# 3DOM-FBK/deep-image-matching

Measured on NVIDIA H100. Metric: image-pairs/sec (SuperPoint+LightGlue, 1024x1024, 2048 kpts), higher is better.
Workload: dtype f16 hi/lo split x3 MMA, f32 accumulate (fp32-class)

## Files before the change

deep-image-matching_b200/csrc/attention.cuh:

```cuda
#pragma once
#include "common.cuh"
#include "sm90.cuh"

namespace {

constexpr int kAttnBlk = 64;
constexpr int kAttnTile = 128;
constexpr int kAttnThreads = 9 * 32;

template <int HD, bool SPLIT>
struct AttnGeom {
  static constexpr int kPl = SPLIT ? 2 : 1;
  static constexpr int kAtoms = HD / 64;
  static constexpr int kAtomQ = kAttnTile * 128, kQB = kAtoms * kAtomQ;
  static constexpr int kAtomK = kAttnBlk * 128, kKB = kAtoms * kAtomK;
  static constexpr int kVB = HD * 128;
  static constexpr int kSmem = kPl * (kQB + 2 * (kKB + kVB)) + 256 + 1024;
};

template <int HD, bool SPLIT, class Out>
__device__ __forceinline__ void attn_tile(const CUtensorMap* tmQh, const CUtensorMap* tmQl, const CUtensorMap* tmKh,
                                          const CUtensorMap* tmKl, const CUtensorMap* tmVh, const CUtensorMap* tmVl, int qrow, int krow,
                                          int vrow, int nq, int nk, float scale, float lazy, const Out& out) {
  using namespace sm90;
  using G = AttnGeom<HD, SPLIT>;
  extern __shared__ uint8_t sm_attn_raw[];
  uint8_t* smem = sm_attn_raw + ((1024u - (smem_u32(sm_attn_raw) & 1023u)) & 1023u);
  uint8_t* sQ = smem;
  uint8_t* sK = sQ + G::kPl * G::kQB;
  uint8_t* sV = sK + 2 * G::kPl * G::kKB;
  uint64_t* bars = reinterpret_cast<uint64_t*>(sV + 2 * G::kPl * G::kVB);
  uint64_t *bQ = bars, *kFull = bars + 1, *kEmpty = bars + 3, *vFull = bars + 5, *vEmpty = bars + 7;
  const int tid = threadIdx.x, warp = tid >> 5, lane = tid & 31;
  if (tid == 0) {
    mbar_init(bQ, 1);
    for (int i = 0; i < 2; ++i) {
      mbar_init(&kFull[i], 1);
      mbar_init(&kEmpty[i], 8);
      mbar_init(&vFull[i], 1);
      mbar_init(&vEmpty[i], 8);
    }
    fence_barrier_init();
  }
  __syncthreads();
  const int nblk = (nk + kAttnBlk - 1) / kAttnBlk;

  if (warp == 8) {
    if (nblk > 0 && elect_one()) {
      mbar_expect_tx(bQ, G::kPl * G::kQB);
      for (int at = 0; at < G::kAtoms; ++at) {
        tma_load_2d(sQ + at * G::kAtomQ, tmQh, bQ, at * 64, qrow);
        if (SPLIT) tma_load_2d(sQ + G::kQB + at * G::kAtomQ, tmQl, bQ, at * 64, qrow);
      }
    }
    __syncwarp();
    for (int j = 0; j < nblk; ++j) {
      const int s = j & 1;
      const uint32_t ph = (j >> 1) & 1;
      mbar_wait(&kEmpty[s], ph ^ 1);
      if (elect_one()) {
        mbar_expect_tx(&kFull[s], G::kPl * G::kKB);
        for (int at = 0; at < G::kAtoms; ++at) {
          tma_load_2d(sK + s * G::kPl * G::kKB + at * G::kAtomK, tmKh, &kFull[s], at * 64, krow + j * kAttnBlk);
          if (SPLIT) tma_load_2d(sK + s * G::kPl * G::kKB + G::kKB + at * G::kAtomK, tmKl, &kFull[s], at * 64, krow + j * kAttnBlk);
        }
      }
      __syncwarp();
      mbar_wait(&vEmpty[s], ph ^ 1);
      if (elect_one()) {
        mbar_expect_tx(&vFull[s], G::kPl * G::kVB);
        tma_load_2d(sV + s * G::kPl * G::kVB, tmVh, &vFull[s], j * kAttnBlk, vrow);
        if (SPLIT) tma_load_2d(sV + s * G::kPl * G::kVB + G::kVB, tmVl, &vFull[s], j * kAttnBlk, vrow);
      }
      __syncwarp();
    }
    return;
  }
  const int wg = warp >> 2, w4 = warp & 3;
  const int r0 = 64 * wg + 16 * w4 + (lane >> 2);
  const uint32_t q_wg = smem_u32(sQ) + wg * 64 * 128;
  float o[HD / 2];
#pragma unroll
  for (int i = 0; i < HD / 2; ++i) o[i] = 0.f;
  float m_run[2] = {-INFINITY, -INFINITY}, l_run[2] = {0.f, 0.f};
  const float c2 = scale * 1.4426950408889634f;
  if (nblk > 0) mbar_wait(bQ, 0);
  for (int j = 0; j < nblk; ++j) {
    const int s = j & 1;
    const uint32_t ph = (j >> 1) & 1;
    float sc[kAttnBlk / 2];
    mbar_wait(&kFull[s], ph);
    {
      const uint32_t kb = smem_u32(sK + s * G::kPl * G::kKB);
      wgmma_fence();
#pragma unroll
      for (int kk = 0; kk < 4 * G::kAtoms; ++kk) {
        const uint64_t qh = sdesc_advance_k(make_sdesc_sw128(q_wg + (kk >> 2) * G::kAtomQ), kk & 3);
        const uint64_t kh = sdesc_advance_k(make_sdesc_sw128(kb + (kk >> 2) * G::kAtomK), kk & 3);
        Wgmma<kAttnBlk>::ss(sc, qh, kh, kk != 0);
        if (SPLIT) {
          const uint64_t ql = sdesc_advance_k(make_sdesc_sw128(q_wg + G::kQB + (kk >> 2) * G::kAtomQ), kk & 3);
          const uint64_t kl = sdesc_advance_k(make_sdesc_sw128(kb + G::kKB + (kk >> 2) * G::kAtomK), kk & 3);
          Wgmma<kAttnBlk>::ss(sc, qh, kl, 1);
          Wgmma<kAttnBlk>::ss(sc, ql, kh, 1);
        }
      }
      wgmma_commit();
      wgmma_wait<0>();
      wgmma_fence_regs(sc);
    }
    if (lane == 0) mbar_arrive(&kEmpty[s]);
    const int key0 = j * kAttnBlk + 2 * (lane & 3);
    if (j * kAttnBlk + kAttnBlk > nk) {
#pragma unroll
      for (int i = 0; i < kAttnBlk / 8; ++i)
#pragma unroll
        for (int e = 0; e < 4; ++e)
          if (key0 + 8 * i + (e & 1) >= nk) sc[4 * i + e] = -INFINITY;
    }
    float alpha[2], mc[2];
#pragma unroll
    for (int h = 0; h < 2; ++h) {
      float mx = sc[2 * h];
#pragma unroll
      for (int i = 0; i < kAttnBlk / 8; ++i) mx = fmaxf(mx, fmaxf(sc[4 * i + 2 * h], sc[4 * i + 2 * h + 1]));
      mx = fmaxf(mx, __shfl_xor_sync(0xffffffffu, mx, 1));
      mx = fmaxf(mx, __shfl_xor_sync(0xffffffffu, mx, 2));
      const float m_blk = fmaxf(m_run[h], mx);
      const bool grow = (m_blk - m_run[h]) * c2 > lazy;
      const float m_new = grow ? m_blk : m_run[h];
      alpha[h] = grow ? fast_exp2((m_run[h] - m_new) * c2) : 1.f;
      mc[h] = m_new * c2;
      m_run[h] = m_new;
    }
    float ps[2] = {0.f, 0.f};
#pragma unroll
    for (int i = 0; i < kAttnBlk / 8; ++i)
#pragma unroll
      for (int e = 0; e < 4; ++e) {
        sc[4 * i + e] = fast_exp2(fmaf(sc[4 * i + e], c2, -mc[e >> 1]));
        ps[e >> 1] += sc[4 * i + e];
      }
#pragma unroll
    for (int h = 0; h < 2; ++h) l_run[h] = l_run[h] * alpha[h] + ps[h];
#pragma unroll
    for (int i = 0; i < HD / 8; ++i) {
      o[4 * i] *= alpha[0], o[4 * i + 1] *= alpha[0];
      o[4 * i + 2] *= alpha[1], o[4 * i + 3] *= alpha[1];
    }
    uint32_t ph_[kAttnBlk / 4], pl_[kAttnBlk / 4];
#pragma unroll
    for (int c = 0; c < kAttnBlk / 4; ++c) {
      __half2 h2, l2;
      split2_f32(sc[2 * c], sc[2 * c + 1], h2, l2);
      ph_[c] = *reinterpret_cast<uint32_t*>(&h2);
      pl_[c] = *reinterpret_cast<uint32_t*>(&l2);
    }
    mbar_wait(&vFull[s], ph);
    {
      const uint32_t vb = smem_u32(sV + s * G::kPl * G::kVB);
      const uint64_t v_h = make_sdesc_sw128(vb), v_l = make_sdesc_sw128(vb + G::kVB);
      wgmma_fence();
#pragma unroll
      for (int kk = 0; kk < kAttnBlk / 16; ++kk) {
        const uint32_t ah[4] = {ph_[4 * kk], ph_[4 * kk + 1], ph_[4 * kk + 2], ph_[4 * kk + 3]};
        Wgmma<HD>::rs(o, ah, sdesc_advance_k(v_h, kk), 1);
        if (SPLIT) {
          const uint32_t al[4] = {pl_[4 * kk], pl_[4 * kk + 1], pl_[4 * kk + 2], pl_[4 * kk + 3]};
          Wgmma<HD>::rs(o, ah, sdesc_advance_k(v_l, kk), 1);
          Wgmma<HD>::rs(o, al, sdesc_advance_k(v_h, kk), 1);
        }
      }
      wgmma_commit();
      wgmma_wait<0>();
      wgmma_fence_regs(o);
    }
    if (lane == 0) mbar_arrive(&vEmpty[s]);
  }
  float inv[2];
#pragma unroll
  for (int h = 0; h < 2; ++h) {
    float l = l_run[h];
    l += __shfl_xor_sync(0xffffffffu, l, 1);
    l += __shfl_xor_sync(0xffffffffu, l, 2);
    inv[h] = nblk > 0 ? 1.f / l : 0.f;
  }
#pragma unroll
  for (int i = 0; i < HD / 8; ++i) {
    const int col = 8 * i + 2 * (lane & 3);
    if (r0 < nq) out(r0, col, o[4 * i] * inv[0], o[4 * i + 1] * inv[0]);
    if (r0 + 8 < nq) out(r0 + 8, col, o[4 * i + 2] * inv[1], o[4 * i + 3] * inv[1]);
  }
}

}
```

deep-image-matching_b200/csrc/sm90.cuh:

```cuda
#pragma once
#include <cuda.h>
#include <cuda_fp16.h>
#include <cuda_runtime.h>
#include <stdint.h>

namespace sm90 {

__device__ __forceinline__ uint32_t smem_u32(const void* p) {
  return static_cast<uint32_t>(__cvta_generic_to_shared(p));
}

__device__ __forceinline__ void mbar_init(uint64_t* bar, uint32_t count) {
  asm volatile("mbarrier.init.shared::cta.b64 [%0], %1;" ::"r"(smem_u32(bar)), "r"(count) : "memory");
}
__device__ __forceinline__ void fence_barrier_init() {
  asm volatile("fence.mbarrier_init.release.cluster;" ::: "memory");
}
__device__ __forceinline__ void mbar_expect_tx(uint64_t* bar, uint32_t bytes) {
  asm volatile("mbarrier.arrive.expect_tx.shared::cta.b64 _, [%0], %1;" ::"r"(smem_u32(bar)), "r"(bytes) : "memory");
}
__device__ __forceinline__ void mbar_arrive(uint64_t* bar) {
  asm volatile("mbarrier.arrive.shared::cta.b64 _, [%0];" ::"r"(smem_u32(bar)) : "memory");
}
__device__ __forceinline__ bool mbar_try_wait(uint64_t* bar, uint32_t parity) {
  uint32_t ok;
  asm volatile(
      "{\n\t.reg .pred p;\n\t"
      "mbarrier.try_wait.parity.shared::cta.b64 p, [%1], %2;\n\t"
      "selp.u32 %0, 1, 0, p;\n\t}"
      : "=r"(ok)
      : "r"(smem_u32(bar)), "r"(parity)
      : "memory");
  return ok != 0;
}
__device__ __forceinline__ void mbar_wait(uint64_t* bar, uint32_t parity) {
  if (mbar_try_wait(bar, parity)) return;
  uint32_t polls = 0;
  long long t0 = 0;
  while (!mbar_try_wait(bar, parity)) {
    if ((++polls & 0x3ffu) == 0) {
      const long long now = clock64();
      if (t0 == 0) t0 = now;
      if (now - t0 > 8000000000LL) {
        __trap();
      }
    }
  }
}

__device__ __forceinline__ float fast_exp2(float x) {
  float y;
  asm("ex2.approx.ftz.f32 %0, %1;" : "=f"(y) : "f"(x));
  return y;
}

__device__ __forceinline__ bool elect_one() {
  uint32_t pred;
  asm volatile(
      "{\n\t.reg .pred p;\n\t"
      "elect.sync _|p, 0xffffffff;\n\t"
      "selp.u32 %0, 1, 0, p;\n\t}"
      : "=r"(pred));
  return pred != 0;
}

__device__ __forceinline__ void fence_proxy_async_smem() {
  asm volatile("fence.proxy.async.shared::cta;" ::: "memory");
}
template <int N>
__device__ __forceinline__ void setmaxnreg_dec() {
  asm volatile("setmaxnreg.dec.sync.aligned.u32 %0;" ::"n"(N));
}
template <int N>
__device__ __forceinline__ void setmaxnreg_inc() {
  asm volatile("setmaxnreg.inc.sync.aligned.u32 %0;" ::"n"(N));
}
__device__ __forceinline__ void named_bar_sync(int id, int threads) {
  asm volatile("bar.sync %0, %1;" ::"r"(id), "r"(threads) : "memory");
}

__device__ __forceinline__ void tma_prefetch_desc(const CUtensorMap* m) {
  asm volatile("prefetch.tensormap [%0];" ::"l"(reinterpret_cast<uint64_t>(m)) : "memory");
}
__device__ __forceinline__ void tma_load_2d(void* dst, const CUtensorMap* m, uint64_t* bar, int c0, int c1) {
  asm volatile(
      "cp.async.bulk.tensor.2d.shared::cluster.global.mbarrier::complete_tx::bytes [%0], [%1, {%3, %4}], [%2];" ::"r"(
          smem_u32(dst)),
      "l"(reinterpret_cast<uint64_t>(m)), "r"(smem_u32(bar)), "r"(c0), "r"(c1)
      : "memory");
}
__device__ __forceinline__ void tma_load_4d(void* dst, const CUtensorMap* m, uint64_t* bar, int c0, int c1, int c2, int c3) {
  asm volatile(
      "cp.async.bulk.tensor.4d.shared::cluster.global.mbarrier::complete_tx::bytes [%0], [%1, {%3, %4, %5, %6}], [%2];" ::
          "r"(smem_u32(dst)),
      "l"(reinterpret_cast<uint64_t>(m)), "r"(smem_u32(bar)), "r"(c0), "r"(c1), "r"(c2), "r"(c3)
      : "memory");
}

__device__ __forceinline__ void tma_prefetch_2d(const CUtensorMap* m, int c0, int c1) {
  asm volatile("cp.async.bulk.prefetch.tensor.2d.L2.global.tile [%0, {%1, %2}];" ::"l"(reinterpret_cast<uint64_t>(m)), "r"(c0), "r"(c1)
               : "memory");
}
__device__ __forceinline__ void tma_prefetch_4d(const CUtensorMap* m, int c0, int c1, int c2, int c3) {
  asm volatile("cp.async.bulk.prefetch.tensor.4d.L2.global.tile [%0, {%1, %2, %3, %4}];" ::"l"(reinterpret_cast<uint64_t>(m)), "r"(c0),
               "r"(c1), "r"(c2), "r"(c3)
               : "memory");
}

constexpr uint32_t kLayoutSw128 = 1, kLayoutSw64 = 2;
__device__ __forceinline__ uint64_t make_sdesc(uint32_t saddr, uint32_t sbo_bytes, uint32_t layout) {
  uint64_t d = 0;
  d |= static_cast<uint64_t>((saddr & 0x3FFFFu) >> 4);
  d |= static_cast<uint64_t>(1) << 16;
  d |= static_cast<uint64_t>(sbo_bytes >> 4) << 32;
  d |= static_cast<uint64_t>(layout) << 62;
  return d;
}
__device__ __forceinline__ uint64_t make_sdesc_sw128(uint32_t saddr) { return make_sdesc(saddr, 1024, kLayoutSw128); }
__device__ __forceinline__ uint64_t sdesc_advance_k(uint64_t d, int k16) { return d + static_cast<uint64_t>(k16 * 2); }

__device__ __forceinline__ void wgmma_fence() { asm volatile("wgmma.fence.sync.aligned;" ::: "memory"); }
__device__ __forceinline__ void wgmma_commit() { asm volatile("wgmma.commit_group.sync.aligned;" ::: "memory"); }
template <int N>
__device__ __forceinline__ void wgmma_wait() {
  asm volatile("wgmma.wait_group.sync.aligned %0;" ::"n"(N) : "memory");
}
template <int N>
__device__ __forceinline__ void wgmma_fence_regs(float (&d)[N]) {
#pragma unroll
  for (int i = 0; i < N; ++i) asm volatile("" : "+f"(d[i])::"memory");
}

template <int N>
struct Wgmma;

template <>
struct Wgmma<64> {
  static __device__ __forceinline__ void ss(float* d, uint64_t a, uint64_t b, int scale_d) {
    asm volatile(
        "{\n\t.reg .pred p;\n\t"
        "setp.ne.b32 p, %34, 0;\n\t"
        "wgmma.mma_async.sync.aligned.m64n64k16.f32.f16.f16 {%0, %1, %2, %3, %4, %5, %6, %7, %8, %9, %10, %11, %12, %13, %14, %15, %16, %17, %18, %19, %20, %21, %22, %23, %24, %25, %26, %27, %28, %29, %30, %31}, %32, %33, p, 1, 1, 0, 0;\n\t}"
        : "+f"(d[0]), "+f"(d[1]), "+f"(d[2]), "+f"(d[3]), "+f"(d[4]), "+f"(d[5]), "+f"(d[6]), "+f"(d[7]), "+f"(d[8]), "+f"(d[9]), "+f"(d[10]), "+f"(d[11]), "+f"(d[12]), "+f"(d[13]), "+f"(d[14]), "+f"(d[15]), "+f"(d[16]), "+f"(d[17]), "+f"(d[18]), "+f"(d[19]), "+f"(d[20]), "+f"(d[21]), "+f"(d[22]), "+f"(d[23]), "+f"(d[24]), "+f"(d[25]), "+f"(d[26]), "+f"(d[27]), "+f"(d[28]), "+f"(d[29]), "+f"(d[30]), "+f"(d[31])
        : "l"(a), "l"(b), "r"(scale_d));
  }
  static __device__ __forceinline__ void rs(float* d, const uint32_t (&a)[4], uint64_t b, int scale_d) {
    asm volatile(
        "{\n\t.reg .pred p;\n\t"
        "setp.ne.b32 p, %37, 0;\n\t"
        "wgmma.mma_async.sync.aligned.m64n64k16.f32.f16.f16 {%0, %1, %2, %3, %4, %5, %6, %7, %8, %9, %10, %11, %12, %13, %14, %15, %16, %17, %18, %19, %20, %21, %22, %23, %24, %25, %26, %27, %28, %29, %30, %31}, {%32, %33, %34, %35}, %36, p, 1, 1, 0;\n\t}"
        : "+f"(d[0]), "+f"(d[1]), "+f"(d[2]), "+f"(d[3]), "+f"(d[4]), "+f"(d[5]), "+f"(d[6]), "+f"(d[7]), "+f"(d[8]), "+f"(d[9]), "+f"(d[10]), "+f"(d[11]), "+f"(d[12]), "+f"(d[13]), "+f"(d[14]), "+f"(d[15]), "+f"(d[16]), "+f"(d[17]), "+f"(d[18]), "+f"(d[19]), "+f"(d[20]), "+f"(d[21]), "+f"(d[22]), "+f"(d[23]), "+f"(d[24]), "+f"(d[25]), "+f"(d[26]), "+f"(d[27]), "+f"(d[28]), "+f"(d[29]), "+f"(d[30]), "+f"(d[31])
        : "r"(a[0]), "r"(a[1]), "r"(a[2]), "r"(a[3]), "l"(b), "r"(scale_d));
  }
};

template <>
struct Wgmma<128> {
  static __device__ __forceinline__ void ss(float* d, uint64_t a, uint64_t b, int scale_d) {
    asm volatile(
        "{\n\t.reg .pred p;\n\t"
        "setp.ne.b32 p, %66, 0;\n\t"
        "wgmma.mma_async.sync.aligned.m64n128k16.f32.f16.f16 {%0, %1, %2, %3, %4, %5, %6, %7, %8, %9, %10, %11, %12, %13, %14, %15, %16, %17, %18, %19, %20, %21, %22, %23, %24, %25, %26, %27, %28, %29, %30, %31, %32, %33, %34, %35, %36, %37, %38, %39, %40, %41, %42, %43, %44, %45, %46, %47, %48, %49, %50, %51, %52, %53, %54, %55, %56, %57, %58, %59, %60, %61, %62, %63}, %64, %65, p, 1, 1, 0, 0;\n\t}"
        : "+f"(d[0]), "+f"(d[1]), "+f"(d[2]), "+f"(d[3]), "+f"(d[4]), "+f"(d[5]), "+f"(d[6]), "+f"(d[7]), "+f"(d[8]), "+f"(d[9]), "+f"(d[10]), "+f"(d[11]), "+f"(d[12]), "+f"(d[13]), "+f"(d[14]), "+f"(d[15]), "+f"(d[16]), "+f"(d[17]), "+f"(d[18]), "+f"(d[19]), "+f"(d[20]), "+f"(d[21]), "+f"(d[22]), "+f"(d[23]), "+f"(d[24]), "+f"(d[25]), "+f"(d[26]), "+f"(d[27]), "+f"(d[28]), "+f"(d[29]), "+f"(d[30]), "+f"(d[31]), "+f"(d[32]), "+f"(d[33]), "+f"(d[34]), "+f"(d[35]), "+f"(d[36]), "+f"(d[37]), "+f"(d[38]), "+f"(d[39]), "+f"(d[40]), "+f"(d[41]), "+f"(d[42]), "+f"(d[43]), "+f"(d[44]), "+f"(d[45]), "+f"(d[46]), "+f"(d[47]), "+f"(d[48]), "+f"(d[49]), "+f"(d[50]), "+f"(d[51]), "+f"(d[52]), "+f"(d[53]), "+f"(d[54]), "+f"(d[55]), "+f"(d[56]), "+f"(d[57]), "+f"(d[58]), "+f"(d[59]), "+f"(d[60]), "+f"(d[61]), "+f"(d[62]), "+f"(d[63])
        : "l"(a), "l"(b), "r"(scale_d));
  }
  static __device__ __forceinline__ void rs(float* d, const uint32_t (&a)[4], uint64_t b, int scale_d) {
    asm volatile(
        "{\n\t.reg .pred p;\n\t"
        "setp.ne.b32 p, %69, 0;\n\t"
        "wgmma.mma_async.sync.aligned.m64n128k16.f32.f16.f16 {%0, %1, %2, %3, %4, %5, %6, %7, %8, %9, %10, %11, %12, %13, %14, %15, %16, %17, %18, %19, %20, %21, %22, %23, %24, %25, %26, %27, %28, %29, %30, %31, %32, %33, %34, %35, %36, %37, %38, %39, %40, %41, %42, %43, %44, %45, %46, %47, %48, %49, %50, %51, %52, %53, %54, %55, %56, %57, %58, %59, %60, %61, %62, %63}, {%64, %65, %66, %67}, %68, p, 1, 1, 0;\n\t}"
        : "+f"(d[0]), "+f"(d[1]), "+f"(d[2]), "+f"(d[3]), "+f"(d[4]), "+f"(d[5]), "+f"(d[6]), "+f"(d[7]), "+f"(d[8]), "+f"(d[9]), "+f"(d[10]), "+f"(d[11]), "+f"(d[12]), "+f"(d[13]), "+f"(d[14]), "+f"(d[15]), "+f"(d[16]), "+f"(d[17]), "+f"(d[18]), "+f"(d[19]), "+f"(d[20]), "+f"(d[21]), "+f"(d[22]), "+f"(d[23]), "+f"(d[24]), "+f"(d[25]), "+f"(d[26]), "+f"(d[27]), "+f"(d[28]), "+f"(d[29]), "+f"(d[30]), "+f"(d[31]), "+f"(d[32]), "+f"(d[33]), "+f"(d[34]), "+f"(d[35]), "+f"(d[36]), "+f"(d[37]), "+f"(d[38]), "+f"(d[39]), "+f"(d[40]), "+f"(d[41]), "+f"(d[42]), "+f"(d[43]), "+f"(d[44]), "+f"(d[45]), "+f"(d[46]), "+f"(d[47]), "+f"(d[48]), "+f"(d[49]), "+f"(d[50]), "+f"(d[51]), "+f"(d[52]), "+f"(d[53]), "+f"(d[54]), "+f"(d[55]), "+f"(d[56]), "+f"(d[57]), "+f"(d[58]), "+f"(d[59]), "+f"(d[60]), "+f"(d[61]), "+f"(d[62]), "+f"(d[63])
        : "r"(a[0]), "r"(a[1]), "r"(a[2]), "r"(a[3]), "l"(b), "r"(scale_d));
  }
};

template <>
struct Wgmma<256> {
  static __device__ __forceinline__ void ss(float* d, uint64_t a, uint64_t b, int scale_d) {
    asm volatile(
        "{\n\t.reg .pred p;\n\t"
        "setp.ne.b32 p, %130, 0;\n\t"
        "wgmma.mma_async.sync.aligned.m64n256k16.f32.f16.f16 {%0, %1, %2, %3, %4, %5, %6, %7, %8, %9, %10, %11, %12, %13, %14, %15, %16, %17, %18, %19, %20, %21, %22, %23, %24, %25, %26, %27, %28, %29, %30, %31, %32, %33, %34, %35, %36, %37, %38, %39, %40, %41, %42, %43, %44, %45, %46, %47, %48, %49, %50, %51, %52, %53, %54, %55, %56, %57, %58, %59, %60, %61, %62, %63, %64, %65, %66, %67, %68, %69, %70, %71, %72, %73, %74, %75, %76, %77, %78, %79, %80, %81, %82, %83, %84, %85, %86, %87, %88, %89, %90, %91, %92, %93, %94, %95, %96, %97, %98, %99, %100, %101, %102, %103, %104, %105, %106, %107, %108, %109, %110, %111, %112, %113, %114, %115, %116, %117, %118, %119, %120, %121, %122, %123, %124, %125, %126, %127}, %128, %129, p, 1, 1, 0, 0;\n\t}"
        : "+f"(d[0]), "+f"(d[1]), "+f"(d[2]), "+f"(d[3]), "+f"(d[4]), "+f"(d[5]), "+f"(d[6]), "+f"(d[7]), "+f"(d[8]), "+f"(d[9]), "+f"(d[10]), "+f"(d[11]), "+f"(d[12]), "+f"(d[13]), "+f"(d[14]), "+f"(d[15]), "+f"(d[16]), "+f"(d[17]), "+f"(d[18]), "+f"(d[19]), "+f"(d[20]), "+f"(d[21]), "+f"(d[22]), "+f"(d[23]), "+f"(d[24]), "+f"(d[25]), "+f"(d[26]), "+f"(d[27]), "+f"(d[28]), "+f"(d[29]), "+f"(d[30]), "+f"(d[31]), "+f"(d[32]), "+f"(d[33]), "+f"(d[34]), "+f"(d[35]), "+f"(d[36]), "+f"(d[37]), "+f"(d[38]), "+f"(d[39]), "+f"(d[40]), "+f"(d[41]), "+f"(d[42]), "+f"(d[43]), "+f"(d[44]), "+f"(d[45]), "+f"(d[46]), "+f"(d[47]), "+f"(d[48]), "+f"(d[49]), "+f"(d[50]), "+f"(d[51]), "+f"(d[52]), "+f"(d[53]), "+f"(d[54]), "+f"(d[55]), "+f"(d[56]), "+f"(d[57]), "+f"(d[58]), "+f"(d[59]), "+f"(d[60]), "+f"(d[61]), "+f"(d[62]), "+f"(d[63]), "+f"(d[64]), "+f"(d[65]), "+f"(d[66]), "+f"(d[67]), "+f"(d[68]), "+f"(d[69]), "+f"(d[70]), "+f"(d[71]), "+f"(d[72]), "+f"(d[73]), "+f"(d[74]), "+f"(d[75]), "+f"(d[76]), "+f"(d[77]), "+f"(d[78]), "+f"(d[79]), "+f"(d[80]), "+f"(d[81]), "+f"(d[82]), "+f"(d[83]), "+f"(d[84]), "+f"(d[85]), "+f"(d[86]), "+f"(d[87]), "+f"(d[88]), "+f"(d[89]), "+f"(d[90]), "+f"(d[91]), "+f"(d[92]), "+f"(d[93]), "+f"(d[94]), "+f"(d[95]), "+f"(d[96]), "+f"(d[97]), "+f"(d[98]), "+f"(d[99]), "+f"(d[100]), "+f"(d[101]), "+f"(d[102]), "+f"(d[103]), "+f"(d[104]), "+f"(d[105]), "+f"(d[106]), "+f"(d[107]), "+f"(d[108]), "+f"(d[109]), "+f"(d[110]), "+f"(d[111]), "+f"(d[112]), "+f"(d[113]), "+f"(d[114]), "+f"(d[115]), "+f"(d[116]), "+f"(d[117]), "+f"(d[118]), "+f"(d[119]), "+f"(d[120]), "+f"(d[121]), "+f"(d[122]), "+f"(d[123]), "+f"(d[124]), "+f"(d[125]), "+f"(d[126]), "+f"(d[127])
        : "l"(a), "l"(b), "r"(scale_d));
  }
  static __device__ __forceinline__ void rs(float* d, const uint32_t (&a)[4], uint64_t b, int scale_d) {
    asm volatile(
        "{\n\t.reg .pred p;\n\t"
        "setp.ne.b32 p, %133, 0;\n\t"
        "wgmma.mma_async.sync.aligned.m64n256k16.f32.f16.f16 {%0, %1, %2, %3, %4, %5, %6, %7, %8, %9, %10, %11, %12, %13, %14, %15, %16, %17, %18, %19, %20, %21, %22, %23, %24, %25, %26, %27, %28, %29, %30, %31, %32, %33, %34, %35, %36, %37, %38, %39, %40, %41, %42, %43, %44, %45, %46, %47, %48, %49, %50, %51, %52, %53, %54, %55, %56, %57, %58, %59, %60, %61, %62, %63, %64, %65, %66, %67, %68, %69, %70, %71, %72, %73, %74, %75, %76, %77, %78, %79, %80, %81, %82, %83, %84, %85, %86, %87, %88, %89, %90, %91, %92, %93, %94, %95, %96, %97, %98, %99, %100, %101, %102, %103, %104, %105, %106, %107, %108, %109, %110, %111, %112, %113, %114, %115, %116, %117, %118, %119, %120, %121, %122, %123, %124, %125, %126, %127}, {%128, %129, %130, %131}, %132, p, 1, 1, 0;\n\t}"
        : "+f"(d[0]), "+f"(d[1]), "+f"(d[2]), "+f"(d[3]), "+f"(d[4]), "+f"(d[5]), "+f"(d[6]), "+f"(d[7]), "+f"(d[8]), "+f"(d[9]), "+f"(d[10]), "+f"(d[11]), "+f"(d[12]), "+f"(d[13]), "+f"(d[14]), "+f"(d[15]), "+f"(d[16]), "+f"(d[17]), "+f"(d[18]), "+f"(d[19]), "+f"(d[20]), "+f"(d[21]), "+f"(d[22]), "+f"(d[23]), "+f"(d[24]), "+f"(d[25]), "+f"(d[26]), "+f"(d[27]), "+f"(d[28]), "+f"(d[29]), "+f"(d[30]), "+f"(d[31]), "+f"(d[32]), "+f"(d[33]), "+f"(d[34]), "+f"(d[35]), "+f"(d[36]), "+f"(d[37]), "+f"(d[38]), "+f"(d[39]), "+f"(d[40]), "+f"(d[41]), "+f"(d[42]), "+f"(d[43]), "+f"(d[44]), "+f"(d[45]), "+f"(d[46]), "+f"(d[47]), "+f"(d[48]), "+f"(d[49]), "+f"(d[50]), "+f"(d[51]), "+f"(d[52]), "+f"(d[53]), "+f"(d[54]), "+f"(d[55]), "+f"(d[56]), "+f"(d[57]), "+f"(d[58]), "+f"(d[59]), "+f"(d[60]), "+f"(d[61]), "+f"(d[62]), "+f"(d[63]), "+f"(d[64]), "+f"(d[65]), "+f"(d[66]), "+f"(d[67]), "+f"(d[68]), "+f"(d[69]), "+f"(d[70]), "+f"(d[71]), "+f"(d[72]), "+f"(d[73]), "+f"(d[74]), "+f"(d[75]), "+f"(d[76]), "+f"(d[77]), "+f"(d[78]), "+f"(d[79]), "+f"(d[80]), "+f"(d[81]), "+f"(d[82]), "+f"(d[83]), "+f"(d[84]), "+f"(d[85]), "+f"(d[86]), "+f"(d[87]), "+f"(d[88]), "+f"(d[89]), "+f"(d[90]), "+f"(d[91]), "+f"(d[92]), "+f"(d[93]), "+f"(d[94]), "+f"(d[95]), "+f"(d[96]), "+f"(d[97]), "+f"(d[98]), "+f"(d[99]), "+f"(d[100]), "+f"(d[101]), "+f"(d[102]), "+f"(d[103]), "+f"(d[104]), "+f"(d[105]), "+f"(d[106]), "+f"(d[107]), "+f"(d[108]), "+f"(d[109]), "+f"(d[110]), "+f"(d[111]), "+f"(d[112]), "+f"(d[113]), "+f"(d[114]), "+f"(d[115]), "+f"(d[116]), "+f"(d[117]), "+f"(d[118]), "+f"(d[119]), "+f"(d[120]), "+f"(d[121]), "+f"(d[122]), "+f"(d[123]), "+f"(d[124]), "+f"(d[125]), "+f"(d[126]), "+f"(d[127])
        : "r"(a[0]), "r"(a[1]), "r"(a[2]), "r"(a[3]), "l"(b), "r"(scale_d));
  }
};

__device__ __forceinline__ uint32_t sw128_offset(int row, int col) {
  return static_cast<uint32_t>(row * 128 + ((((col >> 3) ^ row) & 7) << 4) + ((col & 7) << 1));
}

}
```

Baseline: 221.9.

## Pipeline attention S and PV wgmmas with ping-pong warpgroup scheduling

Restructures the attention consumer loop in FlashAttention-3 style. Each iteration now issues the QK^T wgmma for block j together with the PV wgmma for block j-1, so the softmax of block j runs while the PV matmul is still in flight. Named barriers make the two warpgroups alternate their MMA issue, Q is held in registers via ldmatrix when the head dim is 64, and the O rescale is skipped when no row max changed. It also adds an early exit when there are no keys. The cost is higher register pressure from the extra live fragments, plus barrier coordination that could serialize or deadlock if the warpgroups' block counts diverge.

After: 227.7 (median of 6 runs). +2.6%, better.

```diff
diff --git a/deep-image-matching_b200/csrc/attention.cuh b/deep-image-matching_b200/csrc/attention.cuh
--- a/deep-image-matching_b200/csrc/attention.cuh
+++ b/deep-image-matching_b200/csrc/attention.cuh
@@ -16,6 +16,7 @@
   static constexpr int kAtomK = kAttnBlk * 128, kKB = kAtoms * kAtomK;
   static constexpr int kVB = HD * 128;
   static constexpr int kSmem = kPl * (kQB + 2 * (kKB + kVB)) + 256 + 1024;
+  static constexpr bool kQReg = HD == 64;
 };
 
 template <int HD, bool SPLIT, class Out>
@@ -78,38 +79,76 @@
   }
   const int wg = warp >> 2, w4 = warp & 3;
   const int r0 = 64 * wg + 16 * w4 + (lane >> 2);
-  const uint32_t q_wg = smem_u32(sQ) + wg * 64 * 128;
   float o[HD / 2];
 #pragma unroll
   for (int i = 0; i < HD / 2; ++i) o[i] = 0.f;
   float m_run[2] = {-INFINITY, -INFINITY}, l_run[2] = {0.f, 0.f};
   const float c2 = scale * 1.4426950408889634f;
-  if (nblk > 0) mbar_wait(bQ, 0);
-  for (int j = 0; j < nblk; ++j) {
-    const int s = j & 1;
-    const uint32_t ph = (j >> 1) & 1;
-    float sc[kAttnBlk / 2];
-    mbar_wait(&kFull[s], ph);
-    {
-      const uint32_t kb = smem_u32(sK + s * G::kPl * G::kKB);
-      wgmma_fence();
-#pragma unroll
-      for (int kk = 0; kk < 4 * G::kAtoms; ++kk) {
+  if (nblk == 0) {
+#pragma unroll
+    for (int i = 0; i < HD / 8; ++i) {
+      const int col = 8 * i + 2 * (lane & 3);
+      if (r0 < nq) out(r0, col, 0.f, 0.f);
+      if (r0 + 8 < nq) out(r0 + 8, col, 0.f, 0.f);
+    }
+    return;
+  }
+  const uint32_t q_wg = smem_u32(sQ) + wg * 64 * 128;
+  uint32_t qf[G::kQReg ? G::kPl : 1][4 * G::kAtoms][4];
+  mbar_wait(bQ, 0);
+  if constexpr (G::kQReg) {
+    const int qr = 64 * wg + 16 * w4 + (lane & 15), qc = 8 * (lane >> 4);
+#pragma unroll
+    for (int pl = 0; pl < G::kPl; ++pl)
+#pragma unroll
+      for (int kk = 0; kk < 4 * G::kAtoms; ++kk)
+        ldmatrix_x4(qf[pl][kk], smem_u32(sQ + pl * G::kQB + (kk >> 2) * G::kAtomQ) + sw128_offset(qr, 16 * (kk & 3) + qc));
+  }
+  float sc[kAttnBlk / 2];
+  uint32_t ph_[kAttnBlk / 4], pl_[kAttnBlk / 4];
+  float alpha[2];
+  auto issue_s = [&](int j) {
+    mbar_wait(&kFull[j & 1], (j >> 1) & 1);
+    const uint32_t kb = smem_u32(sK + (j & 1) * G::kPl * G::kKB);
+#pragma unroll
+    for (int kk = 0; kk < 4 * G::kAtoms; ++kk) {
+      const uint64_t kh = sdesc_advance_k(make_sdesc_sw128(kb + (kk >> 2) * G::kAtomK), kk & 3);
+      const uint64_t kl = sdesc_advance_k(make_sdesc_sw128(kb + G::kKB + (kk >> 2) * G::kAtomK), kk & 3);
+      if constexpr (G::kQReg) {
+        Wgmma<kAttnBlk>::rs(sc, qf[0][kk], kh, kk != 0);
+        if (SPLIT) {
+          Wgmma<kAttnBlk>::rs(sc, qf[0][kk], kl, 1);
+          Wgmma<kAttnBlk>::rs(sc, qf[SPLIT ? 1 : 0][kk], kh, 1);
+        }
+      } else {
         const uint64_t qh = sdesc_advance_k(make_sdesc_sw128(q_wg + (kk >> 2) * G::kAtomQ), kk & 3);
-        const uint64_t kh = sdesc_advance_k(make_sdesc_sw128(kb + (kk >> 2) * G::kAtomK), kk & 3);
+        const uint64_t ql = sdesc_advance_k(make_sdesc_sw128(q_wg + G::kQB + (kk >> 2) * G::kAtomQ), kk & 3);
         Wgmma<kAttnBlk>::ss(sc, qh, kh, kk != 0);
         if (SPLIT) {
-          const uint64_t ql = sdesc_advance_k(make_sdesc_sw128(q_wg + G::kQB + (kk >> 2) * G::kAtomQ), kk & 3);
-          const uint64_t kl = sdesc_advance_k(make_sdesc_sw128(kb + G::kKB + (kk >> 2) * G::kAtomK), kk & 3);
           Wgmma<kAttnBlk>::ss(sc, qh, kl, 1);
           Wgmma<kAttnBlk>::ss(sc, ql, kh, 1);
         }
       }
-      wgmma_commit();
-      wgmma_wait<0>();
-      wgmma_fence_regs(sc);
-    }
-    if (lane == 0) mbar_arrive(&kEmpty[s]);
+    }
+    wgmma_commit();
+  };
+  auto issue_pv = [&](int j) {
+    mbar_wait(&vFull[j & 1], (j >> 1) & 1);
+    const uint32_t vb = smem_u32(sV + (j & 1) * G::kPl * G::kVB);
+    const uint64_t v_h = make_sdesc_sw128(vb), v_l = make_sdesc_sw128(vb + G::kVB);
+#pragma unroll
+    for (int kk = 0; kk < kAttnBlk / 16; ++kk) {
+      const uint32_t ah[4] = {ph_[4 * kk], ph_[4 * kk + 1], ph_[4 * kk + 2], ph_[4 * kk + 3]};
+      Wgmma<HD>::rs(o, ah, sdesc_advance_k(v_h, kk), 1);
+      if (SPLIT) {
+        const uint32_t al[4] = {pl_[4 * kk], pl_[4 * kk + 1], pl_[4 * kk + 2], pl_[4 * kk + 3]};
+        Wgmma<HD>::rs(o, ah, sdesc_advance_k(v_l, kk), 1);
+        Wgmma<HD>::rs(o, al, sdesc_advance_k(v_h, kk), 1);
+      }
+    }
+    wgmma_commit();
+  };
+  auto softmax = [&](int j) {
     const int key0 = j * kAttnBlk + 2 * (lane & 3);
     if (j * kAttnBlk + kAttnBlk > nk) {
 #pragma unroll
@@ -118,7 +157,7 @@
         for (int e = 0; e < 4; ++e)
           if (key0 + 8 * i + (e & 1) >= nk) sc[4 * i + e] = -INFINITY;
     }
-    float alpha[2], mc[2];
+    float mc[2];
 #pragma unroll
     for (int h = 0; h < 2; ++h) {
       float mx = sc[2 * h];
@@ -143,12 +182,15 @@
       }
 #pragma unroll
     for (int h = 0; h < 2; ++h) l_run[h] = l_run[h] * alpha[h] + ps[h];
-#pragma unroll
-    for (int i = 0; i < HD / 8; ++i) {
-      o[4 * i] *= alpha[0], o[4 * i + 1] *= alpha[0];
-      o[4 * i + 2] *= alpha[1], o[4 * i + 3] *= alpha[1];
-    }
-    uint32_t ph_[kAttnBlk / 4], pl_[kAttnBlk / 4];
+  };
+  auto rescale_and_split = [&]() {
+    if (__any_sync(0xffffffffu, alpha[0] != 1.f || alpha[1] != 1.f)) {
+#pragma unroll
+      for (int i = 0; i < HD / 8; ++i) {
+        o[4 * i] *= alpha[0], o[4 * i + 1] *= alpha[0];
+        o[4 * i + 2] *= alpha[1], o[4 * i + 3] *= alpha[1];
+      }
+    }
 #pragma unroll
     for (int c = 0; c < kAttnBlk / 4; ++c) {
       __half2 h2, l2;
@@ -156,34 +198,46 @@
       ph_[c] = *reinterpret_cast<uint32_t*>(&h2);
       pl_[c] = *reinterpret_cast<uint32_t*>(&l2);
     }
-    mbar_wait(&vFull[s], ph);
-    {
-      const uint32_t vb = smem_u32(sV + s * G::kPl * G::kVB);
-      const uint64_t v_h = make_sdesc_sw128(vb), v_l = make_sdesc_sw128(vb + G::kVB);
-      wgmma_fence();
-#pragma unroll
-      for (int kk = 0; kk < kAttnBlk / 16; ++kk) {
-        const uint32_t ah[4] = {ph_[4 * kk], ph_[4 * kk + 1], ph_[4 * kk + 2], ph_[4 * kk + 3]};
-        Wgmma<HD>::rs(o, ah, sdesc_advance_k(v_h, kk), 1);
-        if (SPLIT) {
-          const uint32_t al[4] = {pl_[4 * kk], pl_[4 * kk + 1], pl_[4 * kk + 2], pl_[4 * kk + 3]};
-          Wgmma<HD>::rs(o, ah, sdesc_advance_k(v_l, kk), 1);
-          Wgmma<HD>::rs(o, al, sdesc_advance_k(v_h, kk), 1);
-        }
-      }
-      wgmma_commit();
-      wgmma_wait<0>();
-      wgmma_fence_regs(o);
-    }
-    if (lane == 0) mbar_arrive(&vEmpty[s]);
-  }
+  };
+  const int bar_me = 1 + wg, bar_other = 2 - wg;
+  if (wg == 1) named_bar_arrive(1, 256);
+  named_bar_sync(bar_me, 256);
+  wgmma_fence();
+  issue_s(0);
+  named_bar_arrive(bar_other, 256);
+  wgmma_wait<0>();
+  wgmma_fence_regs(sc);
+  if (lane == 0) mbar_arrive(&kEmpty[0]);
+  softmax(0);
+  rescale_and_split();
+  for (int j = 1; j < nblk; ++j) {
+    named_bar_sync(bar_me, 256);
+    wgmma_fence();
+    issue_s(j);
+    issue_pv(j - 1);
+    named_bar_arrive(bar_other, 256);
+    wgmma_wait<1>();
+    wgmma_fence_regs(sc);
+    if (lane == 0) mbar_arrive(&kEmpty[j & 1]);
+    softmax(j);
+    wgmma_wait<0>();
+    wgmma_fence_regs(o);
+    if (lane == 0) mbar_arrive(&vEmpty[(j - 1) & 1]);
+    rescale_and_split();
+  }
+  named_bar_sync(bar_me, 256);
+  wgmma_fence();
+  issue_pv(nblk - 1);
+  named_bar_arrive(bar_other, 256);
+  wgmma_wait<0>();
+  wgmma_fence_regs(o);
   float inv[2];
 #pragma unroll
   for (int h = 0; h < 2; ++h) {
     float l = l_run[h];
     l += __shfl_xor_sync(0xffffffffu, l, 1);
     l += __shfl_xor_sync(0xffffffffu, l, 2);
-    inv[h] = nblk > 0 ? 1.f / l : 0.f;
+    inv[h] = 1.f / l;
   }
 #pragma unroll
   for (int i = 0; i < HD / 8; ++i) {
@@ -191,6 +245,7 @@
     if (r0 < nq) out(r0, col, o[4 * i] * inv[0], o[4 * i + 1] * inv[0]);
     if (r0 + 8 < nq) out(r0 + 8, col, o[4 * i + 2] * inv[1], o[4 * i + 3] * inv[1]);
   }
+  if (wg == 0) named_bar_sync(1, 256);
 }
 
 }
diff --git a/deep-image-matching_b200/csrc/sm90.cuh b/deep-image-matching_b200/csrc/sm90.cuh
--- a/deep-image-matching_b200/csrc/sm90.cuh
+++ b/deep-image-matching_b200/csrc/sm90.cuh
@@ -78,6 +78,9 @@
 __device__ __forceinline__ void named_bar_sync(int id, int threads) {
   asm volatile("bar.sync %0, %1;" ::"r"(id), "r"(threads) : "memory");
 }
+__device__ __forceinline__ void named_bar_arrive(int id, int threads) {
+  asm volatile("bar.arrive %0, %1;" ::"r"(id), "r"(threads) : "memory");
+}
 
 __device__ __forceinline__ void tma_prefetch_desc(const CUtensorMap* m) {
   asm volatile("prefetch.tensormap [%0];" ::"l"(reinterpret_cast<uint64_t>(m)) : "memory");
@@ -198,4 +201,11 @@
   return static_cast<uint32_t>(row * 128 + ((((col >> 3) ^ row) & 7) << 4) + ((col & 7) << 1));
 }
 
-}
+__device__ __forceinline__ void ldmatrix_x4(uint32_t (&r)[4], uint32_t saddr) {
+  asm volatile("ldmatrix.sync.aligned.m8n8.x4.shared.b16 {%0, %1, %2, %3}, [%4];"
+               : "=r"(r[0]), "=r"(r[1]), "=r"(r[2]), "=r"(r[3])
+               : "r"(saddr)
+               : "memory");
+}
+
+}
```
